# mazouziwissem/improving_yolov8_CBAM_SwinBlock

Measured on AMD Instinct MI355X. Metric: images/sec fwd+bwd YOLOv8s-CBAM-Swin bs=32 640x640, higher is better.
Workload: dtype bf16; 1 GPU; yolov8s.yaml (nc=1) forward + v8 loss + backward + clip + SGD-nesterov + EMA step, bs=32/GPU 640x640 (CBAM + 2x SwinBlock + SPPF5 + SPPF7); global_batch=32, imgsz=640, parallelism=dp1

## Files before the change

improving_yolov8_cbam_swinblock_amd/csrc/common.h:

```cpp
#pragma once
#include <hip/hip_runtime.h>
#include <stdint.h>
#include <stdio.h>

#include "../../include/ymi.h"

typedef __bf16 bf16_t;
typedef __attribute__((ext_vector_type(8))) __bf16 bf16x8;
typedef __attribute__((ext_vector_type(4))) __bf16 bf16x4;
typedef __attribute__((ext_vector_type(4))) float f32x4;
typedef __attribute__((ext_vector_type(2))) float f32x2;
typedef __attribute__((ext_vector_type(4))) uint32_t u32x4;
typedef __attribute__((ext_vector_type(2))) uint32_t u32x2;

#define YMI_WAVE 64

void ymi_set_error(const char* fmt, ...);
#define YMI_CHECK_ARG(cond, ...)          \
    do {                                  \
        if (!(cond)) {                    \
            ymi_set_error(__VA_ARGS__);   \
            return YMI_EINVAL;            \
        }                                 \
    } while (0)
// ... 12 lines not shown
static inline int64_t ymi_pixels(const ymi_tensor* t) { return t->n * t->h * t->w; }
static inline int ymi_stat_fixed_point_shift(int64_t count) {
    int lg = 0;
    while (((int64_t)1 << lg) < count) ++lg;
    const int sh = 37 - lg;
    return sh < 8 ? 8 : sh > 40 ? 40 : sh;
}
static inline size_t ymi_esize(int dtype) { return dtype == YMI_BF16 ? 2 : 4; }
static inline bool ymi_same_shape(const ymi_tensor* a, const ymi_tensor* b) {
    return a->n == b->n && a->h == b->h && a->w == b->w && a->c == b->c;
}
enum YmiOpt {
    OPT_EW_PPT,
    OPT_EW_CAP,
    OPT_RED_CAP,
    OPT_XCD_SHIFT,
    OPT_ATTN_TILED,
    OPT_WGRAD_BLOCKS,
    OPT_WGRAD_BLOCKS128,
    OPT_IGEMM_TILE_BM,
    OPT_IGEMM_TILE_BN,
    OPT_BN_TAIL,
    OPT_WGRAD_PATCH,
    OPT_COUNT
};
int ymi_opt(int id);
static inline int ew_ppt() { return ymi_opt(OPT_EW_PPT); }
static inline int ew_cap() { return ymi_opt(OPT_EW_CAP); }
const void* ymi_zero_page();

template <typename T> struct ElemTraits;
template <> struct ElemTraits<float> {
    static constexpr int CH = 4;
    static constexpr int DT = YMI_F32;
};
template <> struct ElemTraits<bf16_t> {
    static constexpr int CH = 8;
    static constexpr int DT = YMI_BF16;
};

__device__ __forceinline__ float to_f32(float v) { return v; }
__device__ __forceinline__ float to_f32(bf16_t v) { return (float)v; }
template <typename T> __device__ __forceinline__ T from_f32(float v);
template <> __device__ __forceinline__ float from_f32<float>(float v) { return v; }
template <> __device__ __forceinline__ bf16_t from_f32<bf16_t>(float v) { return (bf16_t)v; }

// ... 169 lines not shown
```

improving_yolov8_cbam_swinblock_amd/csrc/first_conv.hip:

```cpp
#include "common.h"

int ymi_bn_bwd_final(const float* part, int blocks, int C, const float* gamma, const float* beta, const float* mean, const float* inv, float inv_count,
                     float* dgamma, float* dbeta, float* coef, hipStream_t stream);

namespace {

constexpr int FC_TH = 8, FC_TW = 64;
constexpr int FC_PR = 2 * FC_TH + 1;
constexpr int FC_ROWB = (2 * FC_TW + 2) * 8;
constexpr int FC_WG_TILES = 4;

enum { FC_STATS = 0, FC_APPLY = 1, FC_BWD_REDUCE = 2, FC_BWD_WGRAD = 3 };

struct FirstConvArgs {
    const float* img;
    const float* w;
    void* x4;
    void* out;
    int64_t ldout;
    float* partials;
    const float* v0;
    const float* v1;
    const float* v2;
    const float* v3;
    float* slab;
    int act;
    int N, C, H, W, Ho, Wo;
    int tiles_h, tiles_w, total;
};

template <int CTRL> __device__ __forceinline__ float fc_dpp_add(float v) {
    return v + __builtin_bit_cast(float, __builtin_amdgcn_update_dpp(0, __builtin_bit_cast(int, v), CTRL, 0xF, 0xF, true));
}
__device__ __forceinline__ float fc_row16_sum(float v) {
    v = fc_dpp_add<0xB1>(v);
    v = fc_dpp_add<0x4E>(v);
    v = fc_dpp_add<0x141>(v);
    v = fc_dpp_add<0x140>(v);
    return v;
}
__device__ __forceinline__ float fc_act(float x, int act) { return act == YMI_ACT_SILU ? silu_f(x) : x; }
__device__ __forceinline__ float fc_act_grad(float x, int act) { return act == YMI_ACT_SILU ? silu_grad_f(x) : 1.0f; }
__device__ __forceinline__ uint32_t fc_pack2(float lo, float hi) {
    typedef __attribute__((ext_vector_type(2))) __bf16 bf16x2;
    const bf16x2 v = {(bf16_t)lo, (bf16_t)hi};
    return __builtin_bit_cast(uint32_t, v);
}

template <int SW> __device__ __forceinline__ int fc_swz(int row) { return SW == 2 ? ((row >> 3) & 1) : (((row >> 1) & 1) | (((row >> 3) & 1) << 1)); }
template <int SW> __device__ __forceinline__ bf16x8 fc_tr_load(const char* img, int rowb, int c0, int lane) {
    typedef __attribute__((ext_vector_type(4))) short s16x4;
// ... 142 lines not shown
            c4 = a.v0[4 * CO + tid];
        }
        ctab[tid] = c0; ctab[CO + tid] = c1; ctab[2 * CO + tid] = c2; ctab[3 * CO + tid] = c3; ctab[4 * CO + tid] = c4;
    }
    __syncthreads();
    bf16x8 wf[NCT][2];
#pragma unroll
    for (int ct = 0; ct < NCT; ++ct)
#pragma unroll
        for (int h = 0; h < 2; ++h) wf[ct][h] = *reinterpret_cast<const bf16x8*>(wtab + (ct * 16 + l15) * 64 + 32 * h + 8 * l4);

    float s1[NCT][4], s2[NCT][4];
#pragma unroll
    for (int ct = 0; ct < NCT; ++ct)
#pragma unroll
        for (int r = 0; r < 4; ++r) s1[ct][r] = s2[ct][r] = 0.f;
    f32x4 dwa[3][NCT];
#pragma unroll
    for (int kt = 0; kt < 3; ++kt)
#pragma unroll
        for (int ct = 0; ct < NCT; ++ct) dwa[kt][ct] = f32x4{0.f, 0.f, 0.f, 0.f};

    char* my = stage + ((MODE == FC_APPLY || MODE == FC_BWD_WGRAD) ? wave * STAGEB : 0);
    constexpr int TILES = MODE == FC_BWD_WGRAD ? FC_WG_TILES : 1;
    const int wg_unit = xcd_unit(blockIdx.x, gridDim.x);
#pragma unroll 1
    for (int ti = 0; ti < TILES; ++ti) {
        const int unit = wg_unit * TILES + ti;
        if (unit >= a.total) break;
        const int tw = unit % a.tiles_w;
        const int t2 = unit / a.tiles_w;
        const int th = t2 % a.tiles_h, n = t2 / a.tiles_h;
        const int oh0 = th * FC_TH, ow0 = tw * FC_TW;
        if (ti > 0) __syncthreads();
        if constexpr (MODE == FC_STATS) fc_patch_from_image(a, patch, n, oh0, ow0, tid);
        else fc_patch_from_x4(a, patch, n, oh0, ow0, tid);

#pragma unroll 1
        for (int rr = 0; rr < FC_TH / 4; ++rr) {
            const int ohl = wave + 4 * rr;
            const int oh = oh0 + ohl;
            const bool row_ok = oh < a.Ho;
            const int64_t rowbase = (((int64_t)n * a.Ho + oh) * a.Wo + ow0) * a.ldout;
            [[maybe_unused]] bf16x4 dy_cur[NCT], dy_nxt[NCT];
            [[maybe_unused]] auto load_dy = [&](int mt, bf16x4 (&dst)[NCT]) {
                const bf16_t* dyp = reinterpret_cast<const bf16_t*>(a.out);
                const int owl = mt * 16 + l15;
// ... 138 lines not shown
template <int MODE>
int fc_launch(const FirstConvArgs& a, int64_t cout, unsigned blocks, hipStream_t s) {
    dim3 grid(blocks), blk(256);
    if (cout == 16) hipLaunchKernelGGL((first_conv_kernel<16, MODE>), grid, blk, 0, s, a);
    else if (cout == 32) hipLaunchKernelGGL((first_conv_kernel<32, MODE>), grid, blk, 0, s, a);
    else if (cout == 48) hipLaunchKernelGGL((first_conv_kernel<48, MODE>), grid, blk, 0, s, a);
    else hipLaunchKernelGGL((first_conv_kernel<64, MODE>), grid, blk, 0, s, a);
    YMI_CHECK_LAUNCH("first_conv");
    return YMI_OK;
}

int fc_geometry(FirstConvArgs& a, int64_t n, int64_t c, int64_t h, int64_t w, int64_t cout) {
    YMI_CHECK_ARG(c >= 1 && c <= 4 && (cout == 16 || cout == 32 || cout == 48 || cout == 64), "first_conv: c <= 4 input channels, 16 / 32 / 48 / 64 output channels");
    YMI_CHECK_ARG(a.act == YMI_ACT_SILU || a.act == YMI_ACT_NONE, "first_conv: SiLU or no activation");
    YMI_CHECK_ARG(w % 4 == 0 && h % 2 == 0 && n > 0, "first_conv: even height, width a multiple of 4");
    const int64_t ho = h / 2, wo = w / 2;
    YMI_CHECK_ARG(n * ho * wo * cout < (1ll << 31) && n * h * w * 4 < (1ll << 31), "first_conv: too large for 32-bit indexing");
    a.N = (int)n; a.C = (int)c; a.H = (int)h; a.W = (int)w; a.Ho = (int)ho; a.Wo = (int)wo;
    a.tiles_h = (int)((ho + FC_TH - 1) / FC_TH); a.tiles_w = (int)((wo + FC_TW - 1) / FC_TW);
    a.total = (int)(n * a.tiles_h * a.tiles_w);
    return YMI_OK;
}

}

extern "C" int64_t ymi_first_conv_stat_blocks(int64_t n, int64_t h, int64_t w) {
    const int64_t ho = h / 2, wo = w / 2;
    return n * ((ho + FC_TH - 1) / FC_TH) * ((wo + FC_TW - 1) / FC_TW);
}

extern "C" int ymi_first_conv_bn_act_fwd(const float* img_nchw, int64_t n, int64_t c, int64_t h, int64_t w, const float* weight_oihw, int64_t cout,
                                         const float* gamma, const float* beta, float* running_mean, float* running_var, float momentum, float eps,
                                         int32_t act, const ymi_tensor* x4, const ymi_tensor* out, float* save_mean, float* save_invstd,
                                         void* workspace, size_t workspace_bytes, void* stream) {
    YMI_CHECK_ARG(img_nchw && weight_oihw && ymi_tensor_ok(out) && ymi_tensor_ok(x4) && workspace, "first_conv: bad argument");
    YMI_CHECK_ARG(((uintptr_t)img_nchw & 15) == 0, "first_conv: 16-byte aligned image");
    FirstConvArgs a{};
    a.act = act;
    int rc = fc_geometry(a, n, c, h, w, cout);
    if (rc) return rc;
    YMI_CHECK_ARG(out->dtype == YMI_BF16 && out->n == n && out->h == a.Ho && out->w == a.Wo && out->c == cout && out->ld % 8 == 0 && ((uintptr_t)out->data & 15) == 0,
                  "first_conv: output must be bfloat16 [n, cout, h/2, w/2] NHWC with 16-byte aligned rows");
    YMI_CHECK_ARG(x4->dtype == YMI_BF16 && x4->n == n && x4->h == h && x4->w == w && x4->c == 4 && x4->ld == 4 && ((uintptr_t)x4->data & 15) == 0,
                  "first_conv: the image copy must be dense bfloat16 [n, 4, h, w] NHWC");
    const int64_t blocks = a.total;
    const size_t need = (size_t)(2 * cout + (blocks + 64) * 2 * cout) * sizeof(float);
    if (workspace_bytes < need) {
        ymi_set_error("first_conv: workspace %zu < %zu bytes", workspace_bytes, need);
        return YMI_EWORKSPACE;
    }
    float* scale = reinterpret_cast<float*>(workspace);
    float* shift = scale + cout;
    a.img = img_nchw; a.w = weight_oihw; a.x4 = x4->data; a.partials = shift + cout;
    hipStream_t s = (hipStream_t)stream;
    rc = fc_launch<FC_STATS>(a, cout, (unsigned)blocks, s);
    if (rc) return rc;
    rc = ymi_bn_finalize(a.partials, blocks, n * a.Ho * a.Wo, cout, gamma, beta, running_mean, running_var, momentum, eps, scale, shift, save_mean, save_invstd, stream);
    if (rc) return rc;
    a.out = out->data; a.ldout = out->ld; a.v0 = scale; a.v1 = shift;
    return fc_launch<FC_APPLY>(a, cout, (unsigned)blocks, s);
}

extern "C" int64_t ymi_first_conv_bwd_workspace(int64_t n, int64_t h, int64_t w, int64_t cout) {
    const int64_t blocks = ymi_first_conv_stat_blocks(n, h, w), wgs = (blocks + FC_WG_TILES - 1) / FC_WG_TILES;
    return (int64_t)sizeof(float) * (blocks * 2 * cout + 5 * cout + wgs * cout * 72) + 1024;
}

extern "C" int ymi_first_conv_bn_act_bwd(const ymi_tensor* x4, const float* weight_oihw, int64_t c, int64_t cout, const float* gamma, const float* beta,
                                         const float* save_mean, const float* save_invstd, int32_t act, const ymi_tensor* dout, float* dgamma,
                                         float* dbeta, float* dw_oihw, void* workspace, size_t workspace_bytes, ymi_wgrad_pending* pending, void* stream) {
    YMI_CHECK_ARG(ymi_tensor_ok(x4) && ymi_tensor_ok(dout) && weight_oihw && save_mean && save_invstd && dgamma && dbeta && dw_oihw && workspace, "first_conv_bwd: bad argument");
    FirstConvArgs a{};
    a.act = act;
    int rc = fc_geometry(a, x4->n, c, x4->h, x4->w, cout);
    if (rc) return rc;
    YMI_CHECK_ARG(x4->dtype == YMI_BF16 && x4->c == 4 && x4->ld == 4 && ((uintptr_t)x4->data & 15) == 0, "first_conv_bwd: the image copy must be dense bfloat16 [n, 4, h, w] NHWC");
    YMI_CHECK_ARG(dout->dtype == YMI_BF16 && dout->n == x4->n && dout->h == a.Ho && dout->w == a.Wo && dout->c == cout && dout->ld % 4 == 0 && ((uintptr_t)dout->data & 7) == 0,
                  "first_conv_bwd: dout must be bfloat16 [n, cout, h/2, w/2] NHWC");
    const int64_t blocks = a.total, wgs = (blocks + FC_WG_TILES - 1) / FC_WG_TILES;
    if ((int64_t)workspace_bytes < ymi_first_conv_bwd_workspace(x4->n, x4->h, x4->w, cout)) {
        ymi_set_error("first_conv_bwd: workspace too small");
        return YMI_EWORKSPACE;
    }
    float* part = reinterpret_cast<float*>(workspace);
    float* coef = part + blocks * 2 * cout;
    float* slab = coef + 5 * cout;
    ymi_wgrad_pending* table = reinterpret_cast<ymi_wgrad_pending*>(slab + wgs * cout * 72);
    table = reinterpret_cast<ymi_wgrad_pending*>(((uintptr_t)table + 63) & ~(uintptr_t)63);
    hipStream_t s = (hipStream_t)stream;
    a.w = weight_oihw; a.x4 = x4->data; a.out = dout->data; a.ldout = dout->ld;
    a.partials = part; a.v0 = gamma; a.v1 = beta; a.v2 = save_mean; a.v3 = save_invstd;
    rc = fc_launch<FC_BWD_REDUCE>(a, cout, (unsigned)blocks, s);
    if (rc) return rc;
    rc = ymi_bn_bwd_final(part, (int)blocks, (int)cout, gamma, beta, save_mean, save_invstd, 1.0f / (float)((int64_t)x4->n * a.Ho * a.Wo), dgamma, dbeta, coef, s);
    if (rc) return rc;
    a.v0 = coef; a.slab = slab;
    rc = fc_launch<FC_BWD_WGRAD>(a, cout, (unsigned)wgs, s);
    if (rc) return rc;
    const int64_t elems = cout * 72;
    const int lanes = wgs > 128 ? 32 : wgs > 32 ? 16 : wgs > 8 ? 8 : 4;
    ymi_wgrad_pending rec{slab, dw_oihw, elems, (int32_t)wgs, 72, 8, (int32_t)cout, (int32_t)c, 9, lanes, 0, (int32_t)((elems / 4 + 256 / lanes - 1) / (256 / lanes)), 0};
    if (pending) {
// ... 6 lines not shown
```

improving_yolov8_cbam_swinblock_amd/csrc/runtime.hip:

```cpp
#include <stdarg.h>
#include <string.h>

#include <stdlib.h>

#include "common.h"

static thread_local char g_err[512] = "";

void ymi_set_error(const char* fmt, ...) {
    va_list ap;
    va_start(ap, fmt);
    vsnprintf(g_err, sizeof(g_err), fmt, ap);
    va_end(ap);
}

extern "C" int ymi_version(void) { return YMI_VERSION; }
extern "C" const char* ymi_last_error(void) { return g_err; }

__device__ __attribute__((aligned(256))) unsigned char ymi_zero_page_storage[256];

const void* ymi_zero_page() {
    static thread_local int cached_dev = -1;
    static thread_local void* cached_ptr = nullptr;
    int dev = 0;
    if (hipGetDevice(&dev) != hipSuccess) return nullptr;
    if (dev != cached_dev) {
        void* p = nullptr;
        if (hipGetSymbolAddress(&p, HIP_SYMBOL(ymi_zero_page_storage)) != hipSuccess) return nullptr;
        cached_ptr = p;
        cached_dev = dev;
    }
    return cached_ptr;
}

struct OptEntry {
    const char* name;
    int value;
};
static OptEntry g_opts[OPT_COUNT] = {
    {"ew_ppt", 64}, {"ew_cap", 512}, {"red_cap", 512}, {"xcd_shift", 0}, {"attn_tiled", 0}, {"wgrad_blocks", 1280}, {"wgrad_blocks128", 768},
    {"igemm_tile_bm", 0}, {"igemm_tile_bn", 0}, {"bn_tail", 0}, {"wgrad_patch", 1},
};
static void opts_from_env() {
    for (int i = 0; i < OPT_COUNT; ++i) {
        char env[64] = "YMI_";
        size_t n = 4;
        for (const char* c = g_opts[i].name; *c && n + 1 < sizeof(env); ++c) env[n++] = (char)((*c >= 'a' && *c <= 'z') ? *c - 32 : *c);
        env[n] = 0;
        if (const char* v = getenv(env)) g_opts[i].value = atoi(v);
    }
    if (const char* t = getenv("YMI_IGEMM_TILE")) {
        int bm = 0, bn = 0;
        if (sscanf(t, "%d,%d", &bm, &bn) == 2) {
            g_opts[OPT_IGEMM_TILE_BM].value = bm;
            g_opts[OPT_IGEMM_TILE_BN].value = bn;
        }
    }
}
int ymi_opt(int id) {
    static const bool init = (opts_from_env(), true);
    (void)init;
    return g_opts[id].value;
}
extern "C" int ymi_set_option(const char* name, int64_t value) {
// ... 35 lines not shown
```

improving_yolov8_cbam_swinblock_amd/csrc/wgrad.hip:

```cpp
#include <stdlib.h>

#include <mutex>
#include <type_traits>

#include "common.h"

int ymi_chan_reduce_final(const float* part, int blocks, int C, float* out0, float* out1, hipStream_t stream);
bool ymi_prof_enabled();
int ymi_prof_start(hipStream_t stream, int family, double flop, double bytes, double peak_tflops);
void ymi_prof_stop(hipStream_t stream, int idx);

struct WgradArgs {
    const void* x;
    const void* dy;
    void* slab;
    int slab_bf16;
    float* bias_slab;
    const void* zero;
    int64_t ldx, ldy;
    int Mpix, H, W, Ho, Wo;
    int stride, pad, KW;
    int CoutP, Cin, NG;
    int pix_per_split;
    int nx, ny, splits, xcd_map;
    int pw_shift;
    uint32_t x_bytes, y_bytes;
    uint32_t wo_mul, wo_shr, ho_mul, ho_shr;
};

__device__ __forceinline__ int wg_fast_div(int n, uint32_t mul, uint32_t shr) { return (int)((__umulhi((uint32_t)n, mul) + (uint32_t)n) >> shr); }

typedef const __attribute__((address_space(1))) void* gptr_t;
typedef __attribute__((address_space(3))) void* lptr_t;
typedef __attribute__((ext_vector_type(4))) short s16x4;

constexpr int WG_BM = 64;
constexpr int WG_BN = 128;
constexpr int WG_BK = 32;
constexpr int WG_NS = 2;
constexpr int WG_WAVES = 5;

__device__ __forceinline__ void wg_buffer_to_lds(const void* base, uint32_t bytes, lptr_t dst, uint32_t voff, uint32_t soff) {
#if defined(__HIP_DEVICE_COMPILE__)
    __builtin_amdgcn_raw_ptr_buffer_load_lds(__builtin_amdgcn_make_buffer_rsrc(const_cast<void*>(base), 0, bytes, 0x00020000), dst, 16, voff, soff, 0, 0);
#endif
}
template <typename T> struct WFrag;
__device__ __forceinline__ int wg_swz_y(int row) { return ((row >> 1) & 1) | (((row >> 3) & 1) << 1); }
__device__ __forceinline__ int wg_swz_x(int row) { return (row & 3) | (((row >> 3) & 1) << 2); }
__device__ __forceinline__ int wg_swz_y32(int row) { return (row >> 3) & 1; }
template <int SW> __device__ __forceinline__ int wg_swz(int row) { return SW == 1 ? wg_swz_x(row) : SW == 2 ? wg_swz_y32(row) : wg_swz_y(row); }
template <int BM> struct YSwz { static constexpr int SW = BM == 128 ? 1 : BM == 32 ? 2 : 0; };

template <> struct WFrag<bf16_t> {
    struct Addr { uint32_t lo, hi; };
    template <int SW>
    static __device__ __forceinline__ Addr addr(const char* img, int rowb, int c0, int lane) {
        const int g = lane >> 4, i = lane & 15, q = i >> 2, p = i & 3;
        const int r_lo = 8 * g + q, r_hi = r_lo + 4;
        const int u = (c0 >> 2) + p;
        const int u_lo = u ^ (wg_swz<SW>(r_lo) << 2);
        const int u_hi = u ^ (wg_swz<SW>(r_hi) << 2);
        return Addr{(uint32_t)(uintptr_t)(lptr_t)(img + r_lo * rowb + u_lo * 8), (uint32_t)(uintptr_t)(lptr_t)(img + r_hi * rowb + u_hi * 8)};
// ... 108 lines not shown
        for (int q = 0; q < 32; ++q) {
            a0 += red[(0 * 32 + q) * 33 + cl];
            a1 += red[(1 * 32 + q) * 33 + cl];
        }
        if (r.out0) r.out0[c] = (float)a0;
        if (r.out1) r.out1[c] = (float)a1;
        if (r.coef) {
            const bool second = r.split > 0 && c >= r.split;
            const float* gp = second ? r.gamma2 : r.gamma;
            const float* bp = second ? r.beta2 : r.beta;
            const int pc = second ? c - r.split : c;
            const float ga = gp ? gp[pc] : 1.0f, be = bp ? bp[pc] : 0.0f;
            const float p0 = r.inv[c], p1 = -r.mean[c] * p0;
            const float k1 = (float)a0 * r.inv_count, k2 = (float)a1 * r.inv_count;
            r.coef[0 * r.C + c] = p0 * ga;
            r.coef[1 * r.C + c] = p1 * ga + be;
            r.coef[2 * r.C + c] = ga * p0;
            r.coef[3 * r.C + c] = ga * p0 * p0 * k2;
            r.coef[4 * r.C + c] = ga * p0 * (k1 + p1 * k2);
        }
    }
}

template <typename T, int NS, int BM, bool BIAS = false, bool PATCH = false>
__global__ __launch_bounds__(256, (BM == 128 ? 3 : WG_WAVES)) void wgrad_kernel(WgradArgs a, YmiBnRider rider) {
    constexpr int BNW = WG_BN, NT = 256;
    constexpr int CH = ElemTraits<T>::CH;
    constexpr int ES = (int)sizeof(T);
    constexpr int YCW = BM * ES / 16, XCW = BNW * ES / 16;
    constexpr int YT = WG_BK * YCW < NT ? WG_BK * YCW : NT;
    constexpr int NY = (WG_BK * YCW + NT - 1) / NT, NX = WG_BK * XCW / NT;
    constexpr int WCOLS = BNW / 64, WROWS = (NT / 64) / WCOLS;
    constexpr int YBYTES = WG_BK * BM * ES, XBYTES = WG_BK * BNW * ES;
    constexpr int STAGE = YBYTES + XBYTES;
    static_assert(NY >= 1 && NX >= 1, "tile too small");
    extern __shared__ __attribute__((aligned(16))) char smem[];

    const int tid = threadIdx.x, lane = tid & 63;
    const int wave = __builtin_amdgcn_readfirstlane(tid >> 6);
    const int wr = wave / WCOLS, wc = wave % WCOLS;
    int bx, by, bz;
    if (rider.nwg && (int)blockIdx.x < rider.nwg) {
        wgrad_rider_final(rider, (int)blockIdx.x, smem);
        return;
    }
    if (a.xcd_map) {
        const int id = (int)blockIdx.x - rider.nwg, xcd = id & 7, seq = id >> 3, nxy = a.nx * a.ny;
        const int zi = seq / nxy, t = seq - zi * nxy;
        const int spx = (a.splits + 7) >> 3;
        bz = xcd * spx + zi;
        if (zi >= spx || bz >= a.splits) return;
        by = t / a.nx;
        bx = t - by * a.nx;
    } else {
        bx = blockIdx.x; by = blockIdx.y; bz = blockIdx.z;
    }
    const int j0 = bx * BNW, co0 = by * BM;
    const int m_begin = bz * a.pix_per_split;
    const int m_end = min(a.Mpix, m_begin + a.pix_per_split);
    const T* __restrict__ xg = reinterpret_cast<const T*>(a.x);
    const T* __restrict__ yg = reinterpret_cast<const T*>(a.dy);
    const T* zero = reinterpret_cast<const T*>(a.zero);

    constexpr bool SWZ = std::is_same<T, bf16_t>::value;
    const int ytid = tid % YT;
    const int ycc = SWZ ? ((ytid % YCW) ^ (wg_swz<YSwz<BM>::SW>(ytid / YCW) << 1)) : (ytid % YCW);
    const bool y_cok = co0 + ycc * CH < a.CoutP;
    static_assert(NT / XCW >= 16 || !std::is_same<T, bf16_t>::value, "bf16: a block-wide load covers >= 16 rows, so a thread's rows share the row bits the swizzle uses");
    const int xrow0 = tid / XCW;
    const int xcc = SWZ ? ((tid % XCW) ^ (wg_swz_x(xrow0) << 1)) : (tid % XCW);
    const int j = j0 + xcc * CH;
    const bool x_cok = j < a.NG;
    const int tap = x_cok ? j / a.Cin : 0;
    const int ci = x_cok ? j - tap * a.Cin : 0;
    const int dh = tap / a.KW - a.pad, dw = tap % a.KW - a.pad;
    const int ldx32 = (int)a.ldx, ldy32 = (int)a.ldy;
    const int s_ = a.stride;
    const int q_ = WG_BK / a.Wo, r_ = WG_BK - q_ * a.Wo;
    const uint32_t d_step = (uint32_t)((q_ * s_ * a.W + r_ * s_) * ldx32);
    const uint32_t d_wwrap = (uint32_t)((s_ * a.W - a.Wo * s_) * ldx32);
    const uint32_t d_hwrap = (uint32_t)((a.H * a.W - a.Ho * s_ * a.W) * ldx32);
    const int ws_lim = a.Wo * s_, hs_lim = a.Ho * s_;
// ... 90 lines not shown
            y_off[i] += y_step;
        }
#pragma unroll
        for (int i = 0; i < NX; ++i) {
            const bool ok = x_cok && x_row[i] < left && (unsigned)(x_hs[i] + dh) < (unsigned)a.H && (unsigned)(x_ws[i] + dw) < (unsigned)a.W;
            const T* src = ok ? xg + x_off[i] : zero;
            __builtin_amdgcn_global_load_lds((gptr_t)src, (lptr_t)(Xs + (i * NT + wave * 64) * 16), 16, 0, 0);
            x_ws[i] += r_ * s_;
            x_hs[i] += q_ * s_;
            x_off[i] += d_step;
            if (x_ws[i] >= ws_lim) {
                x_ws[i] -= ws_lim;
                x_hs[i] += s_;
                x_off[i] += d_wwrap;
            }
            while (x_hs[i] >= hs_lim) {
                x_hs[i] -= hs_lim;
                x_off[i] += d_hwrap;
            }
        }
    };

    constexpr int TR = BM / WROWS / 16, TC = 4;
    f32x4 acc[TR][TC];
#pragma unroll
    for (int r = 0; r < TR; ++r)
#pragma unroll
        for (int c = 0; c < TC; ++c) acc[r][c] = f32x4{0.f, 0.f, 0.f, 0.f};

    const bool do_bias = BIAS && bx == 0 && wc == 0;
    f32x4 accb[BIAS ? TR : 1];
#pragma unroll
    for (int r = 0; r < (BIAS ? TR : 1); ++r) accb[r] = f32x4{0.f, 0.f, 0.f, 0.f};
    const int nk = (m_end - m_begin + WG_BK - 1) / WG_BK;
    constexpr int LPT = NY + NX;
#pragma unroll
    for (int s = 0; s < NS - 1; ++s)
        if (s < nk) issue(s, m_begin + s * WG_BK);
    for (int kt = 0; kt < nk; ++kt) {
        if (kt + NS - 2 < nk) wait_vmcnt_barrier<LPT * (NS - 2)>();
        else wait_vmcnt_barrier<0>();
        if (kt + NS - 1 < nk) issue((kt + NS - 1) % NS, m_begin + (kt + NS - 1) * WG_BK);
        const char* Ys = smem + (kt % NS) * STAGE;
        if constexpr (BIAS) WFrag<T>::template step<BM, TR, TC, BNW, true>(Ys, Ys + YBYTES, wr * (BM / WROWS), wc * 64, lane, acc, do_bias, accb);
        else WFrag<T>::template step<BM, TR, TC, BNW, false>(Ys, Ys + YBYTES, wr * (BM / WROWS), wc * 64, lane, acc, false, accb);
    }

    const int64_t slab_off = (int64_t)bz * a.CoutP * a.NG;
    const int l15 = lane & 15, l4 = lane >> 4;
    if (BIAS && do_bias && l4 == 0) {
#pragma unroll
        for (int r = 0; r < (BIAS ? TR : 1); ++r) {
            const int co = co0 + wr * (BM / WROWS) + r * 16 + l15;
            if (co < a.CoutP) a.bias_slab[(int64_t)bz * a.CoutP + co] = accb[r][0];
        }
    }
    if (std::is_same<T, bf16_t>::value && a.slab_bf16) {
        __syncthreads();
        constexpr int SROW = 144;
        constexpr int RP = TR < 2 ? TR : 2;
        char* st = smem + wave * (RP * 16 * SROW);
        bf16_t* slab = reinterpret_cast<bf16_t*>(a.slab) + slab_off;
        const int srow = lane >> 3, sch = lane & 7;
        const int col = j0 + wc * 64 + sch * 8;
#pragma unroll
        for (int r0 = 0; r0 < TR; r0 += RP) {
#pragma unroll
            for (int rr = 0; rr < RP; ++rr)
#pragma unroll
                for (int c = 0; c < TC; ++c) {
                    const bf16x4 v = {(bf16_t)acc[r0 + rr][c][0], (bf16_t)acc[r0 + rr][c][1], (bf16_t)acc[r0 + rr][c][2], (bf16_t)acc[r0 + rr][c][3]};
                    *reinterpret_cast<bf16x4*>(st + (rr * 16 + l15) * SROW + (c * 16 + 4 * l4) * 2) = v;
                }
            __builtin_amdgcn_fence(__ATOMIC_RELEASE, "wavefront");
            __builtin_amdgcn_wave_barrier();
            __builtin_amdgcn_fence(__ATOMIC_ACQUIRE, "wavefront");
#pragma unroll
            for (int k = 0; k < RP * 2; ++k) {
                const int row = k * 8 + srow;
                const uint4 u = *reinterpret_cast<const uint4*>(st + row * SROW + sch * 16);
                const int co = co0 + wr * (BM / WROWS) + r0 * 16 + row;
                if (co < a.CoutP && col < a.NG) *reinterpret_cast<uint4*>(slab + (int64_t)co * a.NG + col) = u;
            }
            __builtin_amdgcn_fence(__ATOMIC_RELEASE, "wavefront");
            __builtin_amdgcn_wave_barrier();
            __builtin_amdgcn_fence(__ATOMIC_ACQUIRE, "wavefront");
        }
    } else if (std::is_same<T, bf16_t>::value) {
        __syncthreads();
        constexpr int SROW = 272;
        char* st = smem + wave * (16 * SROW);
        float* slab = reinterpret_cast<float*>(a.slab) + slab_off;
        const int srow = lane >> 4, sch = lane & 15;
        const int col = j0 + wc * 64 + sch * 4;
#pragma unroll
        for (int r = 0; r < TR; ++r) {
#pragma unroll
            for (int c = 0; c < TC; ++c) *reinterpret_cast<f32x4*>(st + l15 * SROW + (c * 16 + 4 * l4) * 4) = acc[r][c];
            __builtin_amdgcn_fence(__ATOMIC_RELEASE, "wavefront");
            __builtin_amdgcn_wave_barrier();
            __builtin_amdgcn_fence(__ATOMIC_ACQUIRE, "wavefront");
#pragma unroll
            for (int k = 0; k < 4; ++k) {
                const int row = k * 4 + srow;
                const f32x4 u = *reinterpret_cast<const f32x4*>(st + row * SROW + sch * 16);
                const int co = co0 + wr * (BM / WROWS) + r * 16 + row;
                if (co < a.CoutP && col < a.NG) *reinterpret_cast<f32x4*>(slab + (int64_t)co * a.NG + col) = u;
            }
            __builtin_amdgcn_fence(__ATOMIC_RELEASE, "wavefront");
            __builtin_amdgcn_wave_barrier();
            __builtin_amdgcn_fence(__ATOMIC_ACQUIRE, "wavefront");
        }
// ... 121 lines not shown
        else hi = mid - 1;
    }
    const ymi_wgrad_pending e = tab[lo];
    if (e.slab_bf16) reduce_batch_body<true>(e, red);
    else reduce_batch_body<false>(e, red);
}

static void wg_find_divisor(int d, uint32_t* mul, uint32_t* shr) {
    int lg = 0;
    while ((1 << lg) < d) ++lg;
    *mul = (uint32_t)((((uint64_t)1 << 32) * (((uint64_t)1 << lg) - (uint64_t)d)) / (uint64_t)d + 1);
    *shr = (uint32_t)lg;
}

struct WgradPlan {
    int splits, pix_per_split;
    size_t slab_bytes;
};
static int wgrad_bm(int64_t coutp, bool bf16) {
    if (!bf16) return 64;
    if (coutp <= 32) return 32;
    return (coutp >= 128 && coutp % 128 == 0) || coutp >= 256 ? 128 : 64;
}
static WgradPlan wgrad_plan(int64_t mpix, int64_t coutp, int64_t ng, int bm, size_t slab_esize) {
    const int64_t tiles = ((ng + WG_BN - 1) / WG_BN) * ((coutp + bm - 1) / bm);
    const int target64 = ymi_opt(OPT_WGRAD_BLOCKS);
    const int target128 = ymi_opt(OPT_WGRAD_BLOCKS128);
    const int target = bm == 128 ? target128 : target64;
    int64_t s = (target + tiles - 1) / tiles;
    const int64_t smax = (mpix + 255) / 256;
    if (s > smax) s = smax;
    if (s < 1) s = 1;
    if (s >= 8) s = (s + 7) / 8 * 8 <= smax ? (s + 7) / 8 * 8 : s / 8 * 8;
    int64_t pps = (mpix + s - 1) / s;
    pps = (pps + WG_BK - 1) / WG_BK * WG_BK;
    s = (mpix + pps - 1) / pps;
    WgradPlan p;
    p.splits = (int)s;
    p.pix_per_split = (int)pps;
    p.slab_bytes = ((size_t)s * coutp * ng * slab_esize + 255) / 256 * 256;
    return p;
}

static int64_t pad_to(int64_t v, int64_t m) { return (v + m - 1) / m * m; }

extern "C" size_t ymi_conv2d_bwd_weight_workspace(int64_t m_rows, int64_t cout, int64_t cin, int64_t kh, int64_t kw) {
    const int64_t coutp = pad_to(cout, 8), cinp = pad_to(cin, 8);
    WgradPlan p = wgrad_plan(m_rows, coutp, kh * kw * cinp, 64, 4);
    const WgradPlan p128 = wgrad_plan(m_rows, coutp, kh * kw * cinp, 128, 4);
    if (p128.slab_bytes > p.slab_bytes) p = p128;
    return p.slab_bytes + (size_t)(2048 * 2 + 1) * coutp * sizeof(float) + 256;
}

static int wgrad_impl(const ymi_tensor* x, const ymi_tensor* dy, int64_t cout_real, int64_t cin_real, int64_t kh, int64_t kw, int64_t stride,
                      float* dw_oihw, float* dbias, void* workspace, size_t workspace_bytes, ymi_wgrad_pending* pending, void* stream);

struct WgradLaunch {
    WgradArgs a;
    dim3 grid;
    int bm;
    bool bf16;
    hipStream_t s;
    double flop, bytes;
};
static void wgrad_launch(const WgradLaunch& h, const YmiBnRider* rider) {
    YmiBnRider r{};
    dim3 grid = h.grid;
    if (rider && h.a.xcd_map) {
        r = *rider;
        r.nwg = ((rider->C + 31) / 32 + 7) / 8 * 8;
        grid.x += (unsigned)r.nwg;
    }
    const WgradArgs& a = h.a;
    hipStream_t s = h.s;
    int prof = -1;
    if (ymi_prof_enabled()) prof = ymi_prof_start(s, 1, h.flop, h.bytes, h.bf16 ? 2500.0 : 157.3);
#define YMI_WG_LAUNCH(T, BMV, LDS)                                                                                   \
    do {                                                                                                            \
        if (a.pw_shift >= 0) {                                                                                      \
            if (a.bias_slab) hipLaunchKernelGGL((wgrad_kernel<T, WG_NS, BMV, true, true>), grid, dim3(256), (LDS), s, a, r);         \
            else hipLaunchKernelGGL((wgrad_kernel<T, WG_NS, BMV, false, true>), grid, dim3(256), (LDS), s, a, r);               \
        } else if (a.bias_slab) hipLaunchKernelGGL((wgrad_kernel<T, WG_NS, BMV, true>), grid, dim3(256), (LDS), s, a, r);         \
        else hipLaunchKernelGGL((wgrad_kernel<T, WG_NS, BMV, false>), grid, dim3(256), (LDS), s, a, r);                         \
    } while (0)
    if (h.bf16) {
        if (h.bm == 128) YMI_WG_LAUNCH(bf16_t, 128, (size_t)WG_NS * (WG_BK * (128 + WG_BN) * 2));
        else if (h.bm == 32) YMI_WG_LAUNCH(bf16_t, 32, (size_t)WG_NS * (WG_BK * (32 + WG_BN) * 2));
        else YMI_WG_LAUNCH(bf16_t, 64, (size_t)WG_NS * (WG_BK * (64 + WG_BN) * 2));
    } else {
        const size_t lds = 2 * (size_t)(WG_BK * (WG_BM + WG_BN) * 4);
        (void)hipFuncSetAttribute(reinterpret_cast<const void*>(wgrad_kernel<float, 2, 64, false>), hipFuncAttributeMaxDynamicSharedMemorySize, (int)lds);
        (void)hipFuncSetAttribute(reinterpret_cast<const void*>(wgrad_kernel<float, 2, 64, true>), hipFuncAttributeMaxDynamicSharedMemorySize, (int)lds);
        if (a.bias_slab) hipLaunchKernelGGL((wgrad_kernel<float, 2, 64, true>), grid, dim3(256), lds, s, a, r);
        else hipLaunchKernelGGL((wgrad_kernel<float, 2, 64, false>), grid, dim3(256), lds, s, a, r);
    }
#undef YMI_WG_LAUNCH
    ymi_prof_stop(s, prof);
}
static std::mutex g_hold_mu;
static bool g_hold_on = false, g_held_valid = false;
static WgradLaunch g_held;
static void wgrad_flush_held_locked() {
    if (g_held_valid) {
        g_held_valid = false;
        wgrad_launch(g_held, nullptr);
    }
}
bool ymi_wgrad_issue_held(const YmiBnRider* rider, hipStream_t stream) {
    std::lock_guard<std::mutex> lk(g_hold_mu);
    if (!g_held_valid || g_held.s != stream || !g_held.a.xcd_map) return false;
    g_held_valid = false;
    wgrad_launch(g_held, rider);
    return true;
}
extern "C" int ymi_wgrad_hold(int32_t mode) {
    std::lock_guard<std::mutex> lk(g_hold_mu);
    if (mode == 2) {
        g_held_valid = false;
        return YMI_OK;
// ... 47 lines not shown
        hipLaunchKernelGGL(wgrad_table_write_kernel, dim3(1), dim3(64), 0, s, c, m, device_table + base);
    }
    YMI_CHECK_ARG(total < (1ll << 31), "wgrad_reduce_batch: too many workgroups");
    hipLaunchKernelGGL(wgrad_reduce_batch_kernel, dim3((unsigned)total), dim3(256), 0, s, (const ymi_wgrad_pending*)device_table, (int)n);
    YMI_CHECK_LAUNCH("wgrad_reduce_batch");
    return YMI_OK;
}

static int wgrad_impl(const ymi_tensor* x, const ymi_tensor* dy, int64_t cout_real, int64_t cin_real, int64_t kh, int64_t kw, int64_t stride,
                      float* dw_oihw, float* dbias, void* workspace, size_t workspace_bytes, ymi_wgrad_pending* pending, void* stream) {
    YMI_CHECK_ARG(ymi_tensor_ok(x) && ymi_tensor_ok(dy) && dw_oihw && workspace, "conv2d_bwd_weight: bad argument");
    YMI_CHECK_ARG(x->dtype == dy->dtype, "conv2d_bwd_weight: dtype mismatch");
    const int ch = x->dtype == YMI_BF16 ? 8 : 4;
    YMI_CHECK_ARG(x->c % ch == 0 && x->ld % ch == 0 && dy->c % ch == 0 && dy->ld % ch == 0, "conv2d_bwd_weight: channels must be multiples of %d", ch);
    YMI_CHECK_ARG(kh == kw && (kh == 1 || kh == 3) && (stride == 1 || stride == 2), "conv2d_bwd_weight: k in {1,3}, stride in {1,2}");
    const int64_t pad = kh / 2;
    YMI_CHECK_ARG(dy->n == x->n && dy->h == (x->h + 2 * pad - kh) / stride + 1 && dy->w == (x->w + 2 * pad - kw) / stride + 1, "conv2d_bwd_weight: shapes");
    YMI_CHECK_ARG(cout_real <= dy->c && cin_real <= x->c, "conv2d_bwd_weight: real channel counts");
    YMI_CHECK_ARG(ymi_pixels(x) * x->ld < (1ll << 31) && ymi_pixels(dy) * dy->ld < (1ll << 31), "conv2d_bwd_weight: too large");
    const int64_t mpix = ymi_pixels(dy);
    const int64_t ng = kh * kw * x->c;
    const bool bf16 = x->dtype == YMI_BF16;
    const int bm = wgrad_bm(dy->c, bf16), bn = WG_BN;
    WgradPlan p = wgrad_plan(mpix, dy->c, ng, bm, bf16 ? 2 : 4);
    const bool slab_bf16 = bf16 && p.splits >= 16;
    if (bf16 && !slab_bf16) p = wgrad_plan(mpix, dy->c, ng, bm, 4);
    size_t need = p.slab_bytes + (dbias ? (size_t)(2048 * 2 + 1) * dy->c * sizeof(float) : 0);
    if (workspace_bytes < need) {
        ymi_set_error("conv2d_bwd_weight: workspace %zu < %zu bytes", workspace_bytes, need);
        return YMI_EWORKSPACE;
    }
    WgradArgs a{};
    a.x = x->data; a.dy = dy->data; a.slab = workspace; a.slab_bf16 = slab_bf16 ? 1 : 0; a.zero = ymi_zero_page();
    a.bias_slab = dbias ? reinterpret_cast<float*>(reinterpret_cast<char*>(workspace) + p.slab_bytes) : nullptr;
    YMI_CHECK_ARG(!dbias || (size_t)p.splits * dy->c <= (size_t)(2048 * 2 + 1) * dy->c, "conv2d_bwd_weight: too many splits for the bias partials");
    a.ldx = x->ld; a.ldy = dy->ld;
    a.Mpix = (int)mpix; a.H = (int)x->h; a.W = (int)x->w; a.Ho = (int)dy->h; a.Wo = (int)dy->w;
    a.stride = (int)stride; a.pad = (int)pad; a.KW = (int)kw;
    a.CoutP = (int)dy->c; a.Cin = (int)x->c; a.NG = (int)ng; a.pix_per_split = p.pix_per_split;
    wg_find_divisor(a.Wo, &a.wo_mul, &a.wo_shr);
    wg_find_divisor(a.Ho, &a.ho_mul, &a.ho_shr);
    a.nx = (int)((ng + bn - 1) / bn); a.ny = (int)((dy->c + bm - 1) / bm); a.splits = p.splits;
    a.pw_shift = -1;
    {
        const int64_t xb = ymi_pixels(x) * x->ld * ymi_esize(x->dtype), yb = ymi_pixels(dy) * dy->ld * ymi_esize(dy->dtype);
        const int64_t margin = (x->w + 2) * x->ld * (int64_t)ymi_esize(x->dtype);
        if (bf16 && ymi_opt(OPT_WGRAD_PATCH) && xb + margin < (1ll << 31) && yb < (1ll << 31) && mpix % WG_BK == 0) {
            for (int sh = 5; sh >= 0; --sh) {
                const int pw = 1 << sh, ph = WG_BK >> sh;
                if (dy->w % pw == 0 && dy->h % ph == 0) {
                    a.pw_shift = sh;
                    break;
                }
            }
            a.x_bytes = (uint32_t)xb;
            a.y_bytes = (uint32_t)yb;
        }
    }
    a.xcd_map = p.splits >= 8 ? 1 : 0;
    dim3 grid((unsigned)a.nx, (unsigned)a.ny, (unsigned)p.splits);
    if (a.xcd_map) grid = dim3((unsigned)(8 * ((p.splits + 7) / 8) * a.nx * a.ny), 1, 1);
    hipStream_t s = (hipStream_t)stream;
    const double es = (double)ymi_esize(x->dtype);
    WgradLaunch h{a, grid, bm, bf16, s, 2.0 * (double)mpix * (double)dy->c * (double)ng,
                  ((double)ymi_pixels(x) * x->c + (double)mpix * dy->c) * es + (double)dy->c * ng * 4.0};
// ... 34 lines not shown
```

Before: 2759 images/sec.

## Size first-conv wgrad grid by occupancy and add opt-in wave-group split for wgrad

The first-conv weight-gradient pass no longer packs a fixed four tiles per workgroup. It queries CU count and occupancy and sizes the grid to one full round of resident blocks, spreading tiles evenly. The generic wgrad kernel also gains an optional multi-group mode in which several 256-thread groups in one block each reduce a slice of pixels and combine accumulators through LDS, cutting split count and slab traffic. That mode is behind an option that defaults to off. It adds templates, larger LDS footprints and extra barriers.

After: 2764 images/sec (median of 6 runs). Within noise of the previous version (+0.2%).

```diff
diff --git a/improving_yolov8_cbam_swinblock_amd/csrc/common.h b/improving_yolov8_cbam_swinblock_amd/csrc/common.h
--- a/improving_yolov8_cbam_swinblock_amd/csrc/common.h
+++ b/improving_yolov8_cbam_swinblock_amd/csrc/common.h
@@ -58,6 +58,7 @@
     OPT_IGEMM_TILE_BN,
     OPT_BN_TAIL,
     OPT_WGRAD_PATCH,
+    OPT_WGRAD_INSPLIT,
     OPT_COUNT
 };
 int ymi_opt(int id);
diff --git a/improving_yolov8_cbam_swinblock_amd/csrc/first_conv.hip b/improving_yolov8_cbam_swinblock_amd/csrc/first_conv.hip
--- a/improving_yolov8_cbam_swinblock_amd/csrc/first_conv.hip
+++ b/improving_yolov8_cbam_swinblock_amd/csrc/first_conv.hip
@@ -8,7 +8,6 @@
 constexpr int FC_TH = 8, FC_TW = 64;
 constexpr int FC_PR = 2 * FC_TH + 1;
 constexpr int FC_ROWB = (2 * FC_TW + 2) * 8;
-constexpr int FC_WG_TILES = 4;
 
 enum { FC_STATS = 0, FC_APPLY = 1, FC_BWD_REDUCE = 2, FC_BWD_WGRAD = 3 };
 
@@ -27,6 +26,7 @@
     int act;
     int N, C, H, W, Ho, Wo;
     int tiles_h, tiles_w, total;
+    int wg_tiles;
 };
 
 template <int CTRL> __device__ __forceinline__ float fc_dpp_add(float v) {
@@ -215,7 +215,7 @@
         for (int ct = 0; ct < NCT; ++ct) dwa[kt][ct] = f32x4{0.f, 0.f, 0.f, 0.f};
 
     char* my = stage + ((MODE == FC_APPLY || MODE == FC_BWD_WGRAD) ? wave * STAGEB : 0);
-    constexpr int TILES = MODE == FC_BWD_WGRAD ? FC_WG_TILES : 1;
+    const int TILES = MODE == FC_BWD_WGRAD ? a.wg_tiles : 1;
     const int wg_unit = xcd_unit(blockIdx.x, gridDim.x);
 #pragma unroll 1
     for (int ti = 0; ti < TILES; ++ti) {
@@ -400,6 +400,29 @@
     return YMI_OK;
 }
 
+int64_t fc_wgrad_grid(int64_t tiles, int64_t cout, int* wg_tiles) {
+    static int round_of[4] = {0, 0, 0, 0};
+    int& round = round_of[cout / 16 - 1];
+    if (round == 0) {
+        int dev = 0, cus = 0, per_cu = 0;
+        const void* fn = cout == 16 ? reinterpret_cast<const void*>(first_conv_kernel<16, FC_BWD_WGRAD>)
+                       : cout == 32 ? reinterpret_cast<const void*>(first_conv_kernel<32, FC_BWD_WGRAD>)
+                       : cout == 48 ? reinterpret_cast<const void*>(first_conv_kernel<48, FC_BWD_WGRAD>)
+                                    : reinterpret_cast<const void*>(first_conv_kernel<64, FC_BWD_WGRAD>);
+        if (hipGetDevice(&dev) == hipSuccess && hipDeviceGetAttribute(&cus, hipDeviceAttributeMultiprocessorCount, dev) == hipSuccess &&
+            hipOccupancyMaxActiveBlocksPerMultiprocessor(&per_cu, fn, 256, 0) == hipSuccess && cus > 0 && per_cu > 0)
+            round = cus * per_cu;
+        else
+            (void)hipGetLastError();
+    }
+    const int64_t r = round > 0 ? round : tiles;
+    const int64_t per = tiles > r ? (tiles + r - 1) / r : 1;
+    int64_t wgs = (tiles + per - 1) / per;
+    if (wgs >= 8) wgs = (wgs + 7) / 8 * 8;
+    if (wg_tiles) *wg_tiles = (int)per;
+    return wgs;
+}
+
 }
 
 extern "C" int64_t ymi_first_conv_stat_blocks(int64_t n, int64_t h, int64_t w) {
@@ -440,7 +463,8 @@
 }
 
 extern "C" int64_t ymi_first_conv_bwd_workspace(int64_t n, int64_t h, int64_t w, int64_t cout) {
-    const int64_t blocks = ymi_first_conv_stat_blocks(n, h, w), wgs = (blocks + FC_WG_TILES - 1) / FC_WG_TILES;
+    if (!(cout == 16 || cout == 32 || cout == 48 || cout == 64)) return 0;
+    const int64_t blocks = ymi_first_conv_stat_blocks(n, h, w), wgs = fc_wgrad_grid(blocks, cout, nullptr);
     return (int64_t)sizeof(float) * (blocks * 2 * cout + 5 * cout + wgs * cout * 72) + 1024;
 }
 
@@ -455,7 +479,7 @@
     YMI_CHECK_ARG(x4->dtype == YMI_BF16 && x4->c == 4 && x4->ld == 4 && ((uintptr_t)x4->data & 15) == 0, "first_conv_bwd: the image copy must be dense bfloat16 [n, 4, h, w] NHWC");
     YMI_CHECK_ARG(dout->dtype == YMI_BF16 && dout->n == x4->n && dout->h == a.Ho && dout->w == a.Wo && dout->c == cout && dout->ld % 4 == 0 && ((uintptr_t)dout->data & 7) == 0,
                   "first_conv_bwd: dout must be bfloat16 [n, cout, h/2, w/2] NHWC");
-    const int64_t blocks = a.total, wgs = (blocks + FC_WG_TILES - 1) / FC_WG_TILES;
+    const int64_t blocks = a.total, wgs = fc_wgrad_grid(blocks, cout, &a.wg_tiles);
     if ((int64_t)workspace_bytes < ymi_first_conv_bwd_workspace(x4->n, x4->h, x4->w, cout)) {
         ymi_set_error("first_conv_bwd: workspace too small");
         return YMI_EWORKSPACE;
diff --git a/improving_yolov8_cbam_swinblock_amd/csrc/runtime.hip b/improving_yolov8_cbam_swinblock_amd/csrc/runtime.hip
--- a/improving_yolov8_cbam_swinblock_amd/csrc/runtime.hip
+++ b/improving_yolov8_cbam_swinblock_amd/csrc/runtime.hip
@@ -39,7 +39,7 @@
 };
 static OptEntry g_opts[OPT_COUNT] = {
     {"ew_ppt", 64}, {"ew_cap", 512}, {"red_cap", 512}, {"xcd_shift", 0}, {"attn_tiled", 0}, {"wgrad_blocks", 1280}, {"wgrad_blocks128", 768},
-    {"igemm_tile_bm", 0}, {"igemm_tile_bn", 0}, {"bn_tail", 0}, {"wgrad_patch", 1},
+    {"igemm_tile_bm", 0}, {"igemm_tile_bn", 0}, {"bn_tail", 0}, {"wgrad_patch", 1}, {"wgrad_insplit", 0},
 };
 static void opts_from_env() {
     for (int i = 0; i < OPT_COUNT; ++i) {
diff --git a/improving_yolov8_cbam_swinblock_amd/csrc/wgrad.hip b/improving_yolov8_cbam_swinblock_amd/csrc/wgrad.hip
--- a/improving_yolov8_cbam_swinblock_amd/csrc/wgrad.hip
+++ b/improving_yolov8_cbam_swinblock_amd/csrc/wgrad.hip
@@ -23,6 +23,7 @@
     int CoutP, Cin, NG;
     int pix_per_split;
     int nx, ny, splits, xcd_map;
+    int insplit;
     int pw_shift;
     uint32_t x_bytes, y_bytes;
     uint32_t wo_mul, wo_shr, ho_mul, ho_shr;
@@ -39,6 +40,9 @@
 constexpr int WG_BK = 32;
 constexpr int WG_NS = 2;
 constexpr int WG_WAVES = 5;
+constexpr int WG_NS_S = 2;
+constexpr int WG_WAVES_S = 4;
+constexpr int WG_CUS = 256;
 
 __device__ __forceinline__ void wg_buffer_to_lds(const void* base, uint32_t bytes, lptr_t dst, uint32_t voff, uint32_t soff) {
 #if defined(__HIP_DEVICE_COMPILE__)
@@ -193,8 +197,10 @@
     }
 }
 
-template <typename T, int NS, int BM, bool BIAS = false, bool PATCH = false>
-__global__ __launch_bounds__(256, (BM == 128 ? 3 : WG_WAVES)) void wgrad_kernel(WgradArgs a, YmiBnRider rider) {
+constexpr int TR_OF(int bm) { return bm / 2 / 16; }
+
+template <typename T, int NS, int BM, bool BIAS = false, bool PATCH = false, int S = 1>
+__global__ __launch_bounds__(256 * S, (BM == 128 ? 3 : S > 1 ? WG_WAVES_S : WG_WAVES)) void wgrad_kernel(WgradArgs a, YmiBnRider rider) {
     constexpr int BNW = WG_BN, NT = 256;
     constexpr int CH = ElemTraits<T>::CH;
     constexpr int ES = (int)sizeof(T);
@@ -205,14 +211,20 @@
     constexpr int YBYTES = WG_BK * BM * ES, XBYTES = WG_BK * BNW * ES;
     constexpr int STAGE = YBYTES + XBYTES;
     static_assert(NY >= 1 && NX >= 1, "tile too small");
-    extern __shared__ __attribute__((aligned(16))) char smem[];
-
-    const int tid = threadIdx.x, lane = tid & 63;
+    constexpr int RING = NS * STAGE;
+    static_assert(S == 1 || std::is_same<T, bf16_t>::value, "wave groups: bf16 kernels only");
+    static_assert(S == 1 || (TR_OF(BM) * 4 * NT * 16 + (BIAS ? TR_OF(BM) * NT * 4 : 0) <= S * RING), "a group's accumulators must fit in the rings");
+    extern __shared__ __attribute__((aligned(16))) char smem_wg[];
+
+    const int tid = S > 1 ? (int)(threadIdx.x & (NT - 1)) : (int)threadIdx.x, lane = tid & 63;
+    const int grp = S > 1 ? __builtin_amdgcn_readfirstlane((int)(threadIdx.x >> 8)) : 0;
     const int wave = __builtin_amdgcn_readfirstlane(tid >> 6);
+    char* smem = smem_wg + grp * RING;
     const int wr = wave / WCOLS, wc = wave % WCOLS;
     int bx, by, bz;
     if (rider.nwg && (int)blockIdx.x < rider.nwg) {
-        wgrad_rider_final(rider, (int)blockIdx.x, smem);
+        if (S > 1 && threadIdx.x >= NT) return;
+        wgrad_rider_final(rider, (int)blockIdx.x, smem_wg);
         return;
     }
     if (a.xcd_map) {
@@ -227,8 +239,11 @@
         bx = blockIdx.x; by = blockIdx.y; bz = blockIdx.z;
     }
     const int j0 = bx * BNW, co0 = by * BM;
-    const int m_begin = bz * a.pix_per_split;
-    const int m_end = min(a.Mpix, m_begin + a.pix_per_split);
+    const int wm_begin = bz * a.pix_per_split;
+    const int wm_end = min(a.Mpix, wm_begin + a.pix_per_split);
+    const int gpix = a.pix_per_split / S;
+    const int m_begin = S > 1 ? min(wm_end, wm_begin + grp * gpix) : wm_begin;
+    const int m_end = S > 1 ? min(wm_end, m_begin + gpix) : wm_end;
     const T* __restrict__ xg = reinterpret_cast<const T*>(a.x);
     const T* __restrict__ yg = reinterpret_cast<const T*>(a.dy);
     const T* zero = reinterpret_cast<const T*>(a.zero);
@@ -365,6 +380,7 @@
     };
 
     constexpr int TR = BM / WROWS / 16, TC = 4;
+    static_assert(TR == TR_OF(BM), "wave grid");
     f32x4 acc[TR][TC];
 #pragma unroll
     for (int r = 0; r < TR; ++r)
@@ -388,6 +404,37 @@
         if constexpr (BIAS) WFrag<T>::template step<BM, TR, TC, BNW, true>(Ys, Ys + YBYTES, wr * (BM / WROWS), wc * 64, lane, acc, do_bias, accb);
         else WFrag<T>::template step<BM, TR, TC, BNW, false>(Ys, Ys + YBYTES, wr * (BM / WROWS), wc * 64, lane, acc, false, accb);
     }
+    if constexpr (S > 1) {
+        for (int kt = nk; kt < gpix / WG_BK; ++kt) __builtin_amdgcn_s_barrier();
+        __syncthreads();
+        f32x4* cacc = reinterpret_cast<f32x4*>(smem_wg);
+        float* cbias = reinterpret_cast<float*>(smem_wg + TR * TC * NT * 16);
+        for (int g = 1; g < S; ++g) {
+            if (grp == g) {
+#pragma unroll
+                for (int r = 0; r < TR; ++r)
+#pragma unroll
+                    for (int c = 0; c < TC; ++c) cacc[(r * TC + c) * NT + tid] = acc[r][c];
+                if constexpr (BIAS) {
+#pragma unroll
+                    for (int r = 0; r < TR; ++r) cbias[r * NT + tid] = accb[r][0];
+                }
+            }
+            __syncthreads();
+            if (grp == 0) {
+#pragma unroll
+                for (int r = 0; r < TR; ++r)
+#pragma unroll
+                    for (int c = 0; c < TC; ++c) acc[r][c] += cacc[(r * TC + c) * NT + tid];
+                if constexpr (BIAS) {
+#pragma unroll
+                    for (int r = 0; r < TR; ++r) accb[r][0] += cbias[r * NT + tid];
+                }
+            }
+            __syncthreads();
+        }
+        if (grp) return;
+    }
 
     const int64_t slab_off = (int64_t)bz * a.CoutP * a.NG;
     const int l15 = lane & 15, l4 = lane >> 4;
@@ -399,7 +446,7 @@
         }
     }
     if (std::is_same<T, bf16_t>::value && a.slab_bf16) {
-        __syncthreads();
+        if constexpr (S == 1) __syncthreads();
         constexpr int SROW = 144;
         constexpr int RP = TR < 2 ? TR : 2;
         char* st = smem + wave * (RP * 16 * SROW);
@@ -430,7 +477,7 @@
             __builtin_amdgcn_fence(__ATOMIC_ACQUIRE, "wavefront");
         }
     } else if (std::is_same<T, bf16_t>::value) {
-        __syncthreads();
+        if constexpr (S == 1) __syncthreads();
         constexpr int SROW = 272;
         char* st = smem + wave * (16 * SROW);
         float* slab = reinterpret_cast<float*>(a.slab) + slab_off;
@@ -598,18 +645,32 @@
     if (coutp <= 32) return 32;
     return (coutp >= 128 && coutp % 128 == 0) || coutp >= 256 ? 128 : 64;
 }
-static WgradPlan wgrad_plan(int64_t mpix, int64_t coutp, int64_t ng, int bm, size_t slab_esize) {
+static int wgrad_target(int bm, int S) {
+    const int target = ymi_opt(bm == 128 ? OPT_WGRAD_BLOCKS128 : OPT_WGRAD_BLOCKS);
+    return S > 1 && bm != 128 ? target * WG_WAVES_S / WG_WAVES : target;
+}
+static int wgrad_insplit(int64_t mpix, int64_t coutp, int64_t ng, int bm, bool bf16) {
+    if (!bf16) return 1;
+    const int n = ymi_opt(OPT_WGRAD_INSPLIT);
+    int S = 1;
+    if (n >= 1 && (bm == 128 ? (n == 1 || n == 3) : (n == 1 || n == 2 || n == 4))) S = n;
+    if (S == 1) return 1;
+    const int target = wgrad_target(bm, S);
+    if (target < WG_CUS * S) return 1;
     const int64_t tiles = ((ng + WG_BN - 1) / WG_BN) * ((coutp + bm - 1) / bm);
-    const int target64 = ymi_opt(OPT_WGRAD_BLOCKS);
-    const int target128 = ymi_opt(OPT_WGRAD_BLOCKS128);
-    const int target = bm == 128 ? target128 : target64;
+    const int64_t s = (target / S + tiles - 1) / tiles;
+    return s * S * 256 <= mpix ? S : 1;
+}
+static WgradPlan wgrad_plan(int64_t mpix, int64_t coutp, int64_t ng, int bm, size_t slab_esize, int S = 1) {
+    const int64_t tiles = ((ng + WG_BN - 1) / WG_BN) * ((coutp + bm - 1) / bm);
+    const int target = wgrad_target(bm, S) / S;
     int64_t s = (target + tiles - 1) / tiles;
-    const int64_t smax = (mpix + 255) / 256;
+    const int64_t smax = S > 1 ? mpix / (256 * S) : (mpix + 255) / 256;
     if (s > smax) s = smax;
     if (s < 1) s = 1;
     if (s >= 8) s = (s + 7) / 8 * 8 <= smax ? (s + 7) / 8 * 8 : s / 8 * 8;
     int64_t pps = (mpix + s - 1) / s;
-    pps = (pps + WG_BK - 1) / WG_BK * WG_BK;
+    pps = (pps + WG_BK * S - 1) / (WG_BK * S) * (WG_BK * S);
     s = (mpix + pps - 1) / pps;
     WgradPlan p;
     p.splits = (int)s;
@@ -620,11 +681,18 @@
 
 static int64_t pad_to(int64_t v, int64_t m) { return (v + m - 1) / m * m; }
 
+static bool mpix_ok(int64_t mpix, int S) { return mpix >= 256 * S; }
 extern "C" size_t ymi_conv2d_bwd_weight_workspace(int64_t m_rows, int64_t cout, int64_t cin, int64_t kh, int64_t kw) {
     const int64_t coutp = pad_to(cout, 8), cinp = pad_to(cin, 8);
     WgradPlan p = wgrad_plan(m_rows, coutp, kh * kw * cinp, 64, 4);
     const WgradPlan p128 = wgrad_plan(m_rows, coutp, kh * kw * cinp, 128, 4);
     if (p128.slab_bytes > p.slab_bytes) p = p128;
+    for (int S = 2; S <= 4; ++S) {
+        if (mpix_ok(m_rows, S)) {
+            const WgradPlan ps = wgrad_plan(m_rows, coutp, kh * kw * cinp, S == 3 ? 128 : 64, 4, S);
+            if (ps.slab_bytes > p.slab_bytes) p = ps;
+        }
+    }
     return p.slab_bytes + (size_t)(2048 * 2 + 1) * coutp * sizeof(float) + 256;
 }
 
@@ -639,6 +707,10 @@
     hipStream_t s;
     double flop, bytes;
 };
+static bool wgrad_allow_lds(const void* fn, size_t bytes) {
+    if (bytes > 64 * 1024) (void)hipFuncSetAttribute(fn, hipFuncAttributeMaxDynamicSharedMemorySize, (int)bytes);
+    return true;
+}
 static void wgrad_launch(const WgradLaunch& h, const YmiBnRider* rider) {
     YmiBnRider r{};
     dim3 grid = h.grid;
@@ -651,18 +723,37 @@
     hipStream_t s = h.s;
     int prof = -1;
     if (ymi_prof_enabled()) prof = ymi_prof_start(s, 1, h.flop, h.bytes, h.bf16 ? 2500.0 : 157.3);
-#define YMI_WG_LAUNCH(T, BMV, LDS)                                                                                   \
+#define YMI_WG_LAUNCH1(T, BMV, BIASV, PATCHV, SV, LDS)                                                                \
+    do {                                                                                                            \
+        constexpr int NSV = (SV) > 1 ? WG_NS_S : WG_NS;                                                             \
+        static const bool lds_set = wgrad_allow_lds(reinterpret_cast<const void*>(wgrad_kernel<T, NSV, BMV, BIASV, PATCHV, SV>), (SV) * NSV * (LDS)); \
+        (void)lds_set;                                                                                              \
+        hipLaunchKernelGGL((wgrad_kernel<T, NSV, BMV, BIASV, PATCHV, SV>), grid, dim3(256 * (SV)), (SV) * NSV * (LDS), s, a, r);   \
+    } while (0)
+#define YMI_WG_LAUNCH(T, BMV, SV, LDS)                                                                               \
     do {                                                                                                            \
         if (a.pw_shift >= 0) {                                                                                      \
-            if (a.bias_slab) hipLaunchKernelGGL((wgrad_kernel<T, WG_NS, BMV, true, true>), grid, dim3(256), (LDS), s, a, r);         \
-            else hipLaunchKernelGGL((wgrad_kernel<T, WG_NS, BMV, false, true>), grid, dim3(256), (LDS), s, a, r);               \
-        } else if (a.bias_slab) hipLaunchKernelGGL((wgrad_kernel<T, WG_NS, BMV, true>), grid, dim3(256), (LDS), s, a, r);         \
-        else hipLaunchKernelGGL((wgrad_kernel<T, WG_NS, BMV, false>), grid, dim3(256), (LDS), s, a, r);                         \
+            if (a.bias_slab) YMI_WG_LAUNCH1(T, BMV, true, true, SV, LDS);                                           \
+            else YMI_WG_LAUNCH1(T, BMV, false, true, SV, LDS);                                                      \
+        } else if (a.bias_slab) YMI_WG_LAUNCH1(T, BMV, true, false, SV, LDS);                                       \
+        else YMI_WG_LAUNCH1(T, BMV, false, false, SV, LDS);                                                         \
     } while (0)
     if (h.bf16) {
-        if (h.bm == 128) YMI_WG_LAUNCH(bf16_t, 128, (size_t)WG_NS * (WG_BK * (128 + WG_BN) * 2));
-        else if (h.bm == 32) YMI_WG_LAUNCH(bf16_t, 32, (size_t)WG_NS * (WG_BK * (32 + WG_BN) * 2));
-        else YMI_WG_LAUNCH(bf16_t, 64, (size_t)WG_NS * (WG_BK * (64 + WG_BN) * 2));
+        constexpr size_t LDS128 = (size_t)(WG_BK * (128 + WG_BN) * 2), LDS64 = (size_t)(WG_BK * (64 + WG_BN) * 2),
+                         LDS32 = (size_t)(WG_BK * (32 + WG_BN) * 2);
+        const int S = a.insplit;
+        if (h.bm == 128) {
+            if (S == 3) YMI_WG_LAUNCH(bf16_t, 128, 3, LDS128);
+            else YMI_WG_LAUNCH(bf16_t, 128, 1, LDS128);
+        } else if (h.bm == 32) {
+            if (S == 4) YMI_WG_LAUNCH(bf16_t, 32, 4, LDS32);
+            else if (S == 2) YMI_WG_LAUNCH(bf16_t, 32, 2, LDS32);
+            else YMI_WG_LAUNCH(bf16_t, 32, 1, LDS32);
+        } else {
+            if (S == 4) YMI_WG_LAUNCH(bf16_t, 64, 4, LDS64);
+            else if (S == 2) YMI_WG_LAUNCH(bf16_t, 64, 2, LDS64);
+            else YMI_WG_LAUNCH(bf16_t, 64, 1, LDS64);
+        }
     } else {
         const size_t lds = 2 * (size_t)(WG_BK * (WG_BM + WG_BN) * 4);
         (void)hipFuncSetAttribute(reinterpret_cast<const void*>(wgrad_kernel<float, 2, 64, false>), hipFuncAttributeMaxDynamicSharedMemorySize, (int)lds);
@@ -671,6 +762,7 @@
         else hipLaunchKernelGGL((wgrad_kernel<float, 2, 64, false>), grid, dim3(256), lds, s, a, r);
     }
 #undef YMI_WG_LAUNCH
+#undef YMI_WG_LAUNCH1
     ymi_prof_stop(s, prof);
 }
 static std::mutex g_hold_mu;
@@ -764,9 +856,10 @@
     const int64_t ng = kh * kw * x->c;
     const bool bf16 = x->dtype == YMI_BF16;
     const int bm = wgrad_bm(dy->c, bf16), bn = WG_BN;
-    WgradPlan p = wgrad_plan(mpix, dy->c, ng, bm, bf16 ? 2 : 4);
-    const bool slab_bf16 = bf16 && p.splits >= 16;
-    if (bf16 && !slab_bf16) p = wgrad_plan(mpix, dy->c, ng, bm, 4);
+    const int S = wgrad_insplit(mpix, dy->c, ng, bm, bf16);
+    WgradPlan p = wgrad_plan(mpix, dy->c, ng, bm, bf16 ? 2 : 4, S);
+    const bool slab_bf16 = bf16 && (int64_t)p.splits * S >= 16;
+    if (bf16 && !slab_bf16) p = wgrad_plan(mpix, dy->c, ng, bm, 4, S);
     size_t need = p.slab_bytes + (dbias ? (size_t)(2048 * 2 + 1) * dy->c * sizeof(float) : 0);
     if (workspace_bytes < need) {
         ymi_set_error("conv2d_bwd_weight: workspace %zu < %zu bytes", workspace_bytes, need);
@@ -782,7 +875,7 @@
     a.CoutP = (int)dy->c; a.Cin = (int)x->c; a.NG = (int)ng; a.pix_per_split = p.pix_per_split;
     wg_find_divisor(a.Wo, &a.wo_mul, &a.wo_shr);
     wg_find_divisor(a.Ho, &a.ho_mul, &a.ho_shr);
-    a.nx = (int)((ng + bn - 1) / bn); a.ny = (int)((dy->c + bm - 1) / bm); a.splits = p.splits;
+    a.nx = (int)((ng + bn - 1) / bn); a.ny = (int)((dy->c + bm - 1) / bm); a.splits = p.splits; a.insplit = S;
     a.pw_shift = -1;
     {
         const int64_t xb = ymi_pixels(x) * x->ld * ymi_esize(x->dtype), yb = ymi_pixels(dy) * dy->ld * ymi_esize(dy->dtype);
```
